# Polarisjame/DeepFake

Measured on AMD Instinct MI355X. Metric: train clips/sec (32x224x224 video + 16kHz audio) at 1/2/4/8 MI355X, higher is better.
Workload: dtype bf16; 1 GPU; C2: Swin-T video 32x224x224 (window 8x7x7) + SwinV2 mel 224 + wav2vec2-base 4s@16kHz + FusionModel, full train step; global_batch=8, per_gpu_batch=8, parallelism=dp1, hip_graph=True, captured_overlap=False, captured_bn_broadcast=False, branch_streams=3, regularisers=True

## Files before the change

### deepfake_amd/_lib.py

```python
import ctypes as C
import os

import torch

_HERE = os.path.dirname(os.path.abspath(__file__))
LIB_PATH = os.environ.get("DFK_LIB") or os.path.join(_HERE, "libdfk.so")

F32, BF16 = 0, 1


class Drop(C.Structure):
    _fields_ = [("rng", C.c_void_p), ("mode", C.c_int32), ("site", C.c_int32), ("p", C.c_float),
                ("group_rows", C.c_int32), ("shared", C.c_int32)]


class View(C.Structure):
    _fields_ = [("ptr", C.c_void_p), ("ld", C.c_int64), ("bs0", C.c_int64), ("bs1", C.c_int64),
                ("conv_cg", C.c_int32), ("conv_stride", C.c_int32), ("conv_pad", C.c_int32),
                ("conv_rows", C.c_int32)]


class GemmArgs(C.Structure):
    _fields_ = [("a", View), ("b", View), ("c", C.c_void_p), ("bias", C.c_void_p), ("residual", C.c_void_p),
                ("aux", C.c_void_p), ("ldc", C.c_int64), ("cbs0", C.c_int64), ("cbs1", C.c_int64),
# ... 42 lines not shown
class PilResize(C.Structure):
    _fields_ = [("H", C.c_int32), ("W", C.c_int32), ("cin", C.c_int32), ("out_h", C.c_int32), ("out_w", C.c_int32),
                ("xb", C.c_void_p), ("xk", C.c_void_p), ("kx", C.c_int32),
                ("yb", C.c_void_p), ("yk", C.c_void_p), ("ky", C.c_int32)]


class Conv2dGeo(C.Structure):
    _fields_ = [("N", C.c_int32), ("H", C.c_int32), ("W", C.c_int32), ("C", C.c_int32), ("kh", C.c_int32),
                ("kw", C.c_int32), ("sh", C.c_int32), ("sw", C.c_int32), ("ph", C.c_int32), ("pw", C.c_int32),
                ("Ho", C.c_int32), ("Wo", C.c_int32)]


class Im2colArgs(C.Structure):
    _fields_ = [("sb", C.c_int64), ("sc", C.c_int64), ("st", C.c_int64), ("sh", C.c_int64), ("sw", C.c_int64),
                ("B", C.c_int32), ("cin", C.c_int32), ("T", C.c_int32), ("H", C.c_int32), ("W", C.c_int32),
                ("pd", C.c_int32), ("ph", C.c_int32), ("pw", C.c_int32),
                ("Do", C.c_int32), ("Ho", C.c_int32), ("Wo", C.c_int32)]


_VP, _I64, _I32, _F = C.c_void_p, C.c_int64, C.c_int32, C.c_float
SIGNATURES = {
    "dfk_gemm": [C.POINTER(GemmArgs), _VP],
    "dfk_gemm_workspace": [C.POINTER(GemmArgs)],
    "dfk_colsum": [_VP, C.c_int, _I64, _I64, _I64, _VP, _VP],
    "dfk_gemm_mx": [C.POINTER(GemmArgs), C.POINTER(MxOperand), C.POINTER(MxOperand), _VP],
    "dfk_mx_quant": [_VP, C.c_int, _I64, _I64, _I64, C.c_int, _VP, _I64, _VP, _VP],
    "dfk_layernorm_fwd": [_VP, _VP, _VP, _VP, _VP, _VP, _I64, _I32, _F, C.c_int, _VP, C.POINTER(Drop), _VP],
    "dfk_layernorm_bwd": [_VP, _VP, _VP, _VP, _VP, _VP, _VP, _VP, _I64, _I32, C.c_int, C.c_int, _VP,
                          C.POINTER(Drop), _VP, _VP],
    "dfk_layernorm_bwd_workspace": [_I64, _I32],
    "dfk_wattn_fwd": [C.POINTER(WattnArgs), _VP],
    "dfk_wattn_bwd": [C.POINTER(WattnBwdArgs), _VP],
    "dfk_wattn_bwd_workspace": [C.POINTER(WattnArgs)],
    "dfk_wattn_fwd_policy": [C.c_int32, C.c_int64],
    "dfk_wattn_bwd_policy": [C.c_int32, C.c_int32],
    "dfk_wattn_table_workspace": [C.POINTER(WattnArgs)],
    "dfk_wattn_table": [C.POINTER(WattnArgs), _VP],
    "dfk_patch_im2col": [_VP, C.c_int, _VP, C.c_int, C.POINTER(Im2colArgs), _VP],
    "dfk_patch_merge": [_VP, _VP, C.c_int, C.c_int, C.c_int, C.c_int, C.c_int, C.c_int, C.c_int, _VP],
    "dfk_rowmean": [_VP, _VP, C.c_int, C.c_int, C.c_int, C.c_int, C.c_int, _VP],
    "dfk_cast": [_VP, C.c_int, _VP, C.c_int, _I64, _VP],
    "dfk_gelu_bwd": [_VP, _VP, _VP, _I64, C.c_int, _VP],
    "dfk_posconv_wnorm_fwd": [_VP, _VP, C.c_int32, C.c_int32, C.c_int32, _VP, _VP, _VP, _VP, C.c_int, _VP],
    "dfk_posconv_wnorm_bwd": [_VP, _VP, _VP, _VP, C.c_int32, C.c_int32, C.c_int32, _VP, _VP, _VP, _VP],
    "dfk_cosine_qk_fwd": [_VP, _VP, _VP, _F, _I64, C.c_int, C.c_int, C.c_int, _VP],
    "dfk_cosine_qk_bwd": [_VP, _VP, _VP, _VP, _F, _VP, _I64, C.c_int, C.c_int, C.c_int, _VP, _VP],
# ... 112 lines not shown
```

### deepfake_amd/csrc/gemm.hip

```cpp
#include <mutex>

#include "common.h"

namespace {

constexpr int NT = 256;

struct SplitK {
  float* slab;
  uint32_t* cnt;
};

template <typename T> struct GT;
template <> struct GT<bf16raw> { static constexpr int BK = 64, VEC = 8, PADR = 8, PADK = 16; };
template <> struct GT<float> { static constexpr int BK = 32, VEC = 4, PADR = 4, PADK = 4; };

template <typename T, bool KMAJ, int ROWS>
struct Tile {
  static constexpr int TBK = GT<T>::BK;
  static constexpr int STRIDE = KMAJ ? ROWS + GT<T>::PADK : TBK + GT<T>::PADR;
  static constexpr int ELEMS = KMAJ ? TBK * STRIDE : ROWS * STRIDE;
};

template <bool CONV>
// ... 498 lines not shown
__device__ __forceinline__ bf16x8 frag_dma(const bf16raw* img, int r0, int kb, int lane) {
  if constexpr (!KM) {
    const int r = r0 + (lane & 15), c = (kb >> 3) + (lane >> 4);
    return *reinterpret_cast<const bf16x8*>(img + r * 64 + ((c ^ ((r >> 1) & 7)) << 3));
  } else {
    const int li = lane & 15, q = li >> 2, p = li & 3;
    const int k = kb + (lane >> 4) * 8 + q, c = (r0 >> 3) + (p >> 1);
    const bf16raw* lo = img + k * ROWS + ((c ^ kmaj_swz<ROWS>(k)) << 3) + (p & 1) * 4;
    const bf16raw* hi = img + (k + 4) * ROWS + ((c ^ kmaj_swz<ROWS>(k + 4)) << 3) + (p & 1) * 4;
    const short4v a = __builtin_amdgcn_ds_read_tr16_b64_v4i16((lds_short4*)(lo));
    const short4v b = __builtin_amdgcn_ds_read_tr16_b64_v4i16((lds_short4*)(hi));
    short8 u = {a[0], a[1], a[2], a[3], b[0], b[1], b[2], b[3]};
    return __builtin_bit_cast(bf16x8, u);
  }
}

__host__ __device__ __forceinline__ long view_extent(const dfk_view& v, long rows, long cols) {
  if (v.conv_cg > 0) return ((long)(v.conv_rows - 1) * v.ld + v.conv_cg) * 2;
  return ((rows - 1) * v.ld + cols) * 2;
}

constexpr int kRsPartialMin = 32;

template <int WT, int NWM, int NWN, bool AK, bool BKM, int S, bool RS, bool CONV = false>
__global__ __launch_bounds__(NWM * NWN * 64) void gemm_dma_kernel(const dfk_gemm_args g, int kchunk, int evec,
                                                                  SplitK sk) {
  constexpr int NWV = NWM * NWN, BM = NWM * WT, BN = NWN * WT, MI = WT / 16, BK = 64;
  constexpr int STAGE = (BM + BN) * BK;
  constexpr int ES = WT + 4;
  constexpr int SMEM = S * STAGE * 2 > NWV * WT * ES * 4 ? S * STAGE * 2 : NWV * WT * ES * 4;
  constexpr int LPT = Dma<AK, BM, NWV, CONV>::NI + Dma<BKM, BN, NWV, CONV>::NI;
  __shared__ __attribute__((aligned(16))) float smem_f[SMEM / 4];
  bf16raw* smem = reinterpret_cast<bf16raw*>(smem_f);
  const int tid = threadIdx.x, lane = tid & 63;
  const int wave = __builtin_amdgcn_readfirstlane(tid >> 6);
  const int wm = wave / NWN, wn = wave % NWN;
  int tn, tmi, z;
  const int nwg = gridDim.x * gridDim.y;
  if (g.atomic && g.splitk % 8 == 0 && (int)gridDim.z == g.splitk && nwg > 1) {
    const int lin = blockIdx.z * nwg + blockIdx.y * gridDim.x + blockIdx.x;
    const int j = lin >> 3, i = j % nwg;
    z = (j / nwg) * 8 + (lin & 7);
    tn = i % gridDim.x;
    tmi = i / gridDim.x;
  } else {
    const int bid = blockIdx.y * gridDim.x + blockIdx.x;
    const int xcd = bid & 7, q = nwg >> 3, rr = nwg & 7;
    const int nid = (xcd < rr ? xcd * (q + 1) : rr * (q + 1) + (xcd - rr) * q) + (bid >> 3);
    tn = nid % gridDim.x;
    tmi = nid / gridDim.x;
    z = blockIdx.z;
  }
  const int bn = tn * BN, bm = tmi * BM;
  const int split = z % g.splitk;
  z /= g.splitk;
  const int z0 = z / g.nz1, z1 = z % g.nz1;
  const bf16raw* A = reinterpret_cast<const bf16raw*>(g.a.ptr) + z0 * g.a.bs0 + z1 * g.a.bs1;
  const bf16raw* B = reinterpret_cast<const bf16raw*>(g.b.ptr) + z0 * g.b.bs0 + z1 * g.b.bs1;
  const __amdgpu_buffer_rsrc_t ra = __builtin_amdgcn_make_buffer_rsrc(
      const_cast<bf16raw*>(A), (short)0, (int)(AK ? view_extent(g.a, g.K, g.M) : view_extent(g.a, g.M, g.K)), 0x00020000);
  const __amdgpu_buffer_rsrc_t rb = __builtin_amdgcn_make_buffer_rsrc(
      const_cast<bf16raw*>(B), (short)0, (int)(BKM ? view_extent(g.b, g.K, g.N) : view_extent(g.b, g.N, g.K)), 0x00020000);
  const int kbeg = split * kchunk;
  const int kend = min(g.K, kbeg + kchunk);
  const int ntile = kend > kbeg ? (kend - kbeg + BK - 1) / BK : 0;

  auto issue = [&](int kt, bf16raw* st) {
    Dma<AK, BM, NWV, CONV>::issue(ra, g.a, bm, g.M, kt, kend, st, wave, lane);
    Dma<BKM, BN, NWV, CONV>::issue(rb, g.b, bn, g.N, kt, kend, st + BM * BK, wave, lane);
  };

  f32x4 acc[MI][MI];
#pragma unroll
  for (int i = 0; i < MI; ++i)
// ... 54 lines not shown
    }
  }
  if (RS && do_rs && (lane & 15) == 0) {
    float* rsp = g.splitk >= kRsPartialMin && g.ws
                     ? reinterpret_cast<float*>(g.ws) + (g.atomic ? 0L : (long)g.splitk * g.M * g.N) + (long)split * g.M
                     : nullptr;
#pragma unroll
    for (int h = 0; h < MH; ++h) {
      const int mi = h * NWN + wn;
      if (mi < MI)
#pragma unroll
        for (int r = 0; r < 4; ++r) {
          const int row = bm + wm * WT + mi * 16 + (lane >> 4) * 4 + r;
          if (row < g.M) {
            if (rsp) rsp[row] = accr[h][r];
            else atomicAdd(g.rowsum + row, accr[h][r]);
          }
        }
    }
  }
  asm volatile("s_waitcnt vmcnt(0) lgkmcnt(0)" ::: "memory");
  __syncthreads();
  tile_epilogue<bf16raw, WT>(g, smem_f, acc, lane, wave, wm, wn, bm, bn, z, split,
                             (z * (int)gridDim.y + tmi) * (int)gridDim.x + tn, evec, sk);
}

__global__ __launch_bounds__(1024) void rowsum_reduce_kernel(const float* __restrict__ part, int splitk, int M,
                                                             float* __restrict__ rowsum) {
  __shared__ float red[16][64];
  const int c = threadIdx.x & 63, ph = threadIdx.x >> 6;
  const int row = blockIdx.x * 64 + c;
  float a[4] = {0.f, 0.f, 0.f, 0.f};
  if (row < M) {
    int sp = ph;
    for (; sp + 48 < splitk; sp += 64)
#pragma unroll
      for (int u = 0; u < 4; ++u) a[u] += part[(long)(sp + 16 * u) * M + row];
    for (; sp < splitk; sp += 16) a[0] += part[(long)sp * M + row];
  }
  red[ph][c] = (a[0] + a[1]) + (a[2] + a[3]);
  __syncthreads();
  if (ph == 0 && row < M) {
    float t = 0.f;
#pragma unroll
    for (int i = 0; i < 16; ++i) t += red[i][c];
    rowsum[row] += t;
  }
// ... 103 lines not shown
template <int WT, int NWM, int NWN, int S>
void dispatch_dma_s(const dfk_gemm_args& g, dim3 grid, int kchunk, int evec, SplitK sk, hipStream_t s) {
  const dim3 blk(NWM * NWN * 64);
  if (g.a_kmajor) {
    if (g.b_kmajor) {
      if (g.rowsum) hipLaunchKernelGGL((gemm_dma_kernel<WT, NWM, NWN, true, true, S, true>), grid, blk, 0, s, g, kchunk, evec, sk);
      else hipLaunchKernelGGL((gemm_dma_kernel<WT, NWM, NWN, true, true, S, false>), grid, blk, 0, s, g, kchunk, evec, sk);
    }
    else hipLaunchKernelGGL((gemm_dma_kernel<WT, NWM, NWN, true, false, S, false>), grid, blk, 0, s, g, kchunk, evec, sk);
  } else {
    if (g.b_kmajor) hipLaunchKernelGGL((gemm_dma_kernel<WT, NWM, NWN, false, true, S, false>), grid, blk, 0, s, g, kchunk, evec, sk);
    else hipLaunchKernelGGL((gemm_dma_kernel<WT, NWM, NWN, false, false, S, false>), grid, blk, 0, s, g, kchunk, evec, sk);
  }
}

int dma_stages(int wt) {
  static const int s128 = getenv("DFK_DMA_S128") ? atoi(getenv("DFK_DMA_S128")) : 2;
  if (wt == 128) return s128;
  static const int s64 = getenv("DFK_DMA_S64") ? atoi(getenv("DFK_DMA_S64")) : 2;
  static const int s32 = getenv("DFK_DMA_S32") ? atoi(getenv("DFK_DMA_S32")) : 2;
  return wt == 64 ? s64 : s32;
}

void dispatch_dma(const dfk_gemm_args& g, int wt, dim3 grid, int kchunk, int evec, SplitK sk, hipStream_t s) {
  if (g.a.conv_cg > 0 || g.b.conv_cg > 0) {
    if (wt == 32) dispatch_dma_conv<32>(g, grid, kchunk, evec, sk, s);
    else dispatch_dma_conv<64>(g, grid, kchunk, evec, sk, s);
    return;
  }
  static const int sdw = getenv("DFK_DMA_SDW") ? atoi(getenv("DFK_DMA_SDW")) : 2;
  static const int sdw32 = getenv("DFK_DMA_SDW32") ? atoi(getenv("DFK_DMA_SDW32")) : 2;
  const int st = g.a_kmajor && wt == 64 ? sdw : (g.a_kmajor && wt == 32 ? sdw32 : dma_stages(wt));
  static const int s8w = getenv("DFK_DMA_S8W") ? atoi(getenv("DFK_DMA_S8W")) : 2;
  if (wt == 33) {
    if (s8w == 3) dispatch_dma_s<32, 4, 2, 3>(g, grid, kchunk, evec, sk, s);
    else dispatch_dma_s<32, 4, 2, 2>(g, grid, kchunk, evec, sk, s);
    return;
  }
  if (wt == 34) {
    if (s8w == 3) dispatch_dma_s<32, 2, 4, 3>(g, grid, kchunk, evec, sk, s);
    else dispatch_dma_s<32, 2, 4, 2>(g, grid, kchunk, evec, sk, s);
    return;
  }
  if (wt == 128) {
    if (st == 3) dispatch_dma_s<64, 4, 2, 3>(g, grid, kchunk, evec, sk, s);
    else dispatch_dma_s<64, 4, 2, 2>(g, grid, kchunk, evec, sk, s);
  } else if (wt == 64) {
    if (st == 2) dispatch_dma_s<64, 2, 2, 2>(g, grid, kchunk, evec, sk, s);
    else if (st == 4) dispatch_dma_s<64, 2, 2, 4>(g, grid, kchunk, evec, sk, s);
    else dispatch_dma_s<64, 2, 2, 3>(g, grid, kchunk, evec, sk, s);
  } else {
    if (st == 2) dispatch_dma_s<32, 2, 2, 2>(g, grid, kchunk, evec, sk, s);
    else if (st == 4) dispatch_dma_s<32, 2, 2, 4>(g, grid, kchunk, evec, sk, s);
    else dispatch_dma_s<32, 2, 2, 3>(g, grid, kchunk, evec, sk, s);
  }
// ... 351 lines not shown
  static uint32_t* arena[64] = {};
  static long cursor[64] = {};
  std::lock_guard<std::mutex> lock(mu);
  int dev = 0;
  if (hipGetDevice(&dev) != hipSuccess || dev < 0 || dev >= 64) return nullptr;
  if (!arena[dev]) {
    void* p = nullptr;
    if (hipMalloc(&p, kTickets * 4) != hipSuccess) return nullptr;
    if (hipMemsetAsync(p, 0, kTickets * 4, s) != hipSuccess || hipStreamSynchronize(s) != hipSuccess) {
      (void)hipFree(p);
      return nullptr;
    }
    arena[dev] = static_cast<uint32_t*>(p);
  }
  if (cursor[dev] + n > kTickets) cursor[dev] = 0;
  uint32_t* t = arena[dev] + cursor[dev];
  cursor[dev] += (n + 63) & ~63L;
  return t;
}

extern "C" int dfk_gemm(const dfk_gemm_args* g, hipStream_t s) {
  if (!g || g->mx_q) return DFK_EINVAL;
  return g->dtype == DFK_BF16 ? launch<bf16raw>(*g, s) : launch<float>(*g, s);
}

extern "C" int64_t dfk_gemm_workspace(const dfk_gemm_args* g) {
  if (!g) return -1;
  const int autos = g->splitk > 1 && !g->atomic ? g->splitk
                    : (g->dtype == DFK_BF16 ? auto_splitk<bf16raw>(*g) : auto_splitk<float>(*g));
  const bool dmav = g->dtype == DFK_BF16 && dma_ok(*g) && view_vec(g->a, 8) && view_vec(g->b, 8) &&
                    (g->a_kmajor ? g->M : g->K) % 8 == 0 && (g->b_kmajor ? g->N : g->K) % 8 == 0;
  const int64_t rs = !dmav || !g->rowsum ? 0
                     : (g->atomic && g->splitk >= kRsPartialMin ? (int64_t)g->splitk * g->M * 4
                                                                : (autos >= kRsPartialMin ? (int64_t)autos * g->M * 4 : 0));
  if (autos <= 1) return rs;
  return (int64_t)autos * g->nz0 * g->nz1 * g->M * g->N * 4 + rs;
}

extern "C" int dfk_colsum(const void* x, int dtype, int64_t rows, int64_t cols, int64_t ld, float* out,
                          hipStream_t s) {
  if (!x || !out || cols <= 0) return DFK_EINVAL;
  if (rows <= 0) return 0;
  long chunks = rows < 64 ? 1 : std::min<long>(1024, (rows + 63) / 64);
  long rows_per = (rows + chunks - 1) / chunks;
  chunks = (rows + rows_per - 1) / rows_per;
  dim3 grid(dfk_cdiv(cols, 256), (unsigned)chunks);
// ... 74 lines not shown
```

### deepfake_amd/functional.py

```python
import os

import torch

from . import kernels as K


def _orig(p):
    if p is None or hasattr(p, "_dfk_store") or not isinstance(p, torch.Tensor):
        return p
    from .params import PARAM_BY_PTR
    q = PARAM_BY_PTR.get(p.data_ptr())
    return q if q is not None and q.shape == p.shape else p


def compute_weight(p, dtype):
    if p is None:
        return None
    p = _orig(p)
    if p.dtype == dtype:
        return p
    sh = getattr(p, "_dfk_shadow", None)
    if sh is not None and sh.dtype == dtype:
        return sh
    return p.detach().to(dtype)
# ... 14 lines not shown
    p = _orig(p)
    st = _store(p)
    if st is not None and ctx.needs_input_grad[idx] and not _RECOMPUTING[0]:
        st.uses[id(p)] = st.uses.get(id(p), 0) + 1


def grad_sink(p):
    p = _orig(p)
    st = _store(p)
    if st is not None:
        if p.grad is None:
            st.rebind_grads()
        return p.grad
    return _f32_zeros(p)


def grad_done(p, g):
    p = _orig(p)
    st = _store(p)
    if st is None:
        return g
    st.grad_ready(p)
    return None


def checkpoint(fn, *args):
    import contextlib
    import torch.utils.checkpoint as cp

    @contextlib.contextmanager
    def recompute():
        _RECOMPUTING[0] += 1
        try:
            yield
        finally:
            _RECOMPUTING[0] -= 1
    return cp.checkpoint(fn, *args, use_reentrant=False,
                         context_fn=lambda: (contextlib.nullcontext(), recompute()))


def rows2d(x):
    return x.reshape(-1, x.shape[-1])


def mx_weight(p, transpose=False):
    return K.mx_quant(_orig(p).detach(), transpose=transpose)
# ... 15 lines not shown
        else:
            y = K.linear(x, compute_weight(weight, dt), b, act=act, aux=aux, residual=residual, drop=drop)
        grad_use(ctx, 1, weight)
        grad_use(ctx, 2, bias)
        ctx.save_for_backward(x, weight, bias, aux)
        ctx.act, ctx.has_bias, ctx.has_res, ctx.drop, ctx.mx = act, bias is not None, residual is not None, drop, mx
        return y

    @staticmethod
    def backward(ctx, dy):
        x, weight, bias, aux = ctx.saved_tensors
        dy = dy.contiguous()
        dz = K.dropout(dy, ctx.drop) if ctx.drop is not None else dy
        dz = K.gelu_bwd(dz, aux) if ctx.act == 1 else dz
        dx = None
        if ctx.needs_input_grad[0]:
            if ctx.mx:
                dx = K.gemm_mx(K.mx_quant(dz), mx_weight(weight, transpose=True))
            else:
                dx = K.linear_dx(dz, compute_weight(weight, x.dtype))
        dw = db = None
        want_b = ctx.has_bias and ctx.needs_input_grad[2]
        if ctx.needs_input_grad[1]:
            db = grad_sink(bias) if want_b else None
            dw = grad_done(weight, K.linear_dw(dz, x, grad_sink(weight), db=db))
        elif want_b:
            db = K.colsum(dz, grad_sink(bias))
        if want_b:
            db = grad_done(bias, db)
        return dx, dw, db, None, (dy if ctx.has_res else None), None, None


def linear(x, weight, bias=None, act=0, residual=None, drop=None, mx=False):
    shp = x.shape
    x2 = rows2d(x).contiguous()
    y = LinearFn.apply(x2, weight, bias, act, rows2d(residual).contiguous() if residual is not None else None, drop,
                       mx_ok(x2, weight, mx))
    return y.view(*shp[:-1], weight.shape[0])


class GroupLinearFn(torch.autograd.Function):

    @staticmethod
    def forward(ctx, x, st, wspan, wshape, bspan, skip, *params):
        dt = x.dtype
        src = st.shadow if (dt == torch.bfloat16 and st.shadow is not None) else st.flat
        if src.dtype != dt:
            raise RuntimeError("GroupLinearFn: compute dtype has no flat view")
        W = src[wspan[0]:wspan[0] + wspan[1]].view(wshape)
        B = src[bspan[0]:bspan[0] + bspan[1]] if bspan is not None else None
        y = K.linear(x, W, B)
        for i, p in enumerate(params):
            grad_use(ctx, 6 + i, p)
        ctx.save_for_backward(x, *params)
        ctx.st, ctx.wspan, ctx.wshape, ctx.bspan, ctx.skip = st, wspan, wshape, bspan, skip
        if skip:
            return y, x.view_as(x)
        return y

    @staticmethod
    def backward(ctx, dy, dskip=None):
        x, *params = ctx.saved_tensors
        st, (wo, wn), wshape, bspan = ctx.st, ctx.wspan, ctx.wshape, ctx.bspan
        dy = dy.contiguous()
        src = st.shadow if (x.dtype == torch.bfloat16 and st.shadow is not None) else st.flat
        dx = K.linear_dx(dy, src[wo:wo + wn].view(wshape), residual=dskip if ctx.skip else None) \
            if ctx.needs_input_grad[0] else None
        if any(p.grad is None for p in params):
            st.rebind_grads()
        db = st.grad[bspan[0]:bspan[0] + bspan[1]] if bspan is not None else None
        K.linear_dw(dy, x, st.grad[wo:wo + wn].view(wshape), db=db)
        for p in params:
            grad_done(p, None)
        return (dx, None, None, None, None, None) + (None,) * len(params)


def linear_group(x, weights, biases=None, skip=False):
    shp = x.shape
    x2 = rows2d(x).contiguous()
    st = _store(weights[0])
    if st is not None:
        ws = st.group_span(list(weights))
        bs = st.group_span(list(biases)) if biases is not None else None
        if ws is not None and (biases is None or bs is not None):
            wshape = (sum(w.shape[0] for w in weights), weights[0].shape[1])
            ps = list(weights) + [b for b in (biases or []) if not isinstance(b, int)]
            out = GroupLinearFn.apply(x2, st, ws, wshape, bs, skip, *ps)
            if skip:
                return out[0].view(*shp[:-1], wshape[0]), out[1].view(shp)
            return out.view(*shp[:-1], wshape[0])
    W = torch.cat(list(weights)) if len(weights) > 1 else weights[0]
    b = None
    if biases is not None:
        b = torch.cat([torch.zeros(e, device=x.device, dtype=weights[0].dtype) if isinstance(e, int) else e
                       for e in biases])
    y = linear(x, W, b)
# ... 27 lines not shown
        ctx.res_is_input, ctx.skip, ctx.mx = res_is_input, skip, mx
        if skip:
            return y, x.view_as(x)
        return y

    @staticmethod
    def backward(ctx, dy, dskip=None):
        x, w1, b1, w2, b2, pre, h = ctx.saved_tensors
        dy = dy.contiguous()
        dyr = dy
        if ctx.drop_out is not None:
            dy = K.dropout(dy, ctx.drop_out)
        dt = x.dtype
        extra = dyr if ctx.res_is_input else (dskip if ctx.skip else None)
        if ctx.mx:
            dpre, dpreq = K.gemm_mx(K.mx_quant(dy), mx_weight(w2, transpose=True), act=2, aux=pre, drop=ctx.drop_act,
                                    mx_out=True)
            dx = K.gemm_mx(dpreq, mx_weight(w1, transpose=True),
                           residual=extra.contiguous() if extra is not None else None) \
                if ctx.needs_input_grad[0] else None
        else:
            dpre = K.linear_dx(dy, compute_weight(w2, dt), act=2, aux=pre, drop=ctx.drop_act)
            dx = K.linear_dx(dpre, compute_weight(w1, dt), residual=extra) if ctx.needs_input_grad[0] else None
        db2 = grad_sink(b2)
        dw2 = grad_done(w2, K.linear_dw(dy, h, grad_sink(w2), db=db2))
        db2 = grad_done(b2, db2)
        db1 = grad_sink(b1)
        dw1 = grad_done(w1, K.linear_dw(dpre, x, grad_sink(w1), db=db1))
        db1 = grad_done(b1, db1)
        dres = dyr if (ctx.has_res and not ctx.res_is_input) else None
        return dx, dw1, db1, dw2, db2, dres, None, None, None, None, None


def mlp(x, fc1, fc2, residual=None, drop_act=None, drop_out=None, skip=False, mx=False):
    shp = x.shape
    x2 = rows2d(x).contiguous()
    res_is_input = residual is not None and residual is x
    r2 = x2 if res_is_input else (rows2d(residual).contiguous() if residual is not None else None)
    mx = mx_ok(x2, fc1.weight, mx) and fc2.weight.shape[0] % 128 == 0
    out = MlpFn.apply(x2, fc1.weight, fc1.bias, fc2.weight, fc2.bias, r2, drop_act, drop_out, res_is_input, skip, mx)
    if skip:
        y, xs = out
        return y.view(*shp[:-1], fc2.weight.shape[0]), xs.view(shp)
    return out.view(*shp[:-1], fc2.weight.shape[0])


class LayerNormFn(torch.autograd.Function):

    @staticmethod
    def forward(ctx, x, weight, bias, eps, residual=None, drop=None, skip=False):
        dt = x.dtype
        y, mean, rstd = K.layernorm_fwd(x, compute_weight(weight, dt), compute_weight(bias, dt), eps,
# ... 606 lines not shown
```

### deepfake_amd/kernels.py

```python
import ctypes
import math
import os

import torch

from . import _lib as L

_CU_TARGET_BLOCKS = int(os.environ.get("DFK_DW_TARGET", "256"))


def _view(t, ld, bs0=0, bs1=0, conv=None):
    v = L.View()
    v.ptr = t.data_ptr()
    v.ld, v.bs0, v.bs1 = int(ld), int(bs0), int(bs1)
    if conv:
        v.conv_cg, v.conv_stride, v.conv_pad, v.conv_rows = (int(c) for c in conv)
    return v


def gemm(a, a_ld, a_kmajor, b, b_ld, b_kmajor, M, N, K, c, ldc, *, dtype, c_f32=False, bias=None,
         residual=None, ldr=0, aux=None, ldaux=0, act=0, beta=0.0, atomic=False, splitk=1,
         nz=(1, 1), a_bs=(0, 0), b_bs=(0, 0), c_bs=(0, 0), r_bs=(0, 0), a_conv=None, b_conv=None, bias_bs1=0,
         rowsum=None, drop=None, alpha=0.0):
    g = L.GemmArgs()
    if drop is not None:
        g.drop = L.drop(drop, c.device)
    g.bias_bs1 = int(bias_bs1)
    g.a = _view(a, a_ld, *a_bs, conv=a_conv)
    g.b = _view(b, b_ld, *b_bs, conv=b_conv)
    g.c = c.data_ptr()
    g.bias = bias.data_ptr() if bias is not None else None
    g.residual = residual.data_ptr() if residual is not None else None
    g.aux = aux.data_ptr() if aux is not None else None
    g.ldc, g.cbs0, g.cbs1 = int(ldc), int(c_bs[0]), int(c_bs[1])
    g.ldr, g.rbs0, g.rbs1 = int(ldr), int(r_bs[0]), int(r_bs[1])
    g.ldaux = int(ldaux)
    g.M, g.N, g.K = int(M), int(N), int(K)
    g.dtype = dtype
    g.a_kmajor, g.b_kmajor = int(a_kmajor), int(b_kmajor)
    g.c_f32 = int(c_f32)
    g.nz0, g.nz1 = int(nz[0]), int(nz[1])
    g.splitk = int(splitk)
    g.act = int(act)
    g.atomic = int(atomic)
    g.beta = float(beta)
    g.rowsum = rowsum.data_ptr() if rowsum is not None else None
    g.alpha = float(alpha)
    for t in (a, b, c):
        if not t.is_cuda:
            raise RuntimeError("deepfake_amd: tensors must be on the HIP device (no CPU fallback)")
    ws = None
    nbytes = L.lib().dfk_gemm_workspace(g)
    if nbytes > 0:
        ws = torch.empty(nbytes // 4, device=c.device, dtype=torch.float32)
        g.ws = ws.data_ptr()
    L.check(L.lib().dfk_gemm(g, L.stream()), f"gemm M={M} N={N} K={K}")


def linear(x, w, b=None, act=0, aux=None, residual=None, out=None, beta=0.0, drop=None):
    M, K = x.shape
    N = w.shape[0]
    if out is None:
        out = torch.empty(M, N, device=x.device, dtype=x.dtype)
    gemm(x, x.stride(0), False, w, w.stride(0), False, M, N, K, out, out.stride(0), dtype=L.dt(x), bias=b,
         residual=residual, ldr=residual.stride(0) if residual is not None else 0, aux=aux,
         ldaux=aux.stride(0) if aux is not None else 0, act=act, beta=beta, drop=drop)
    return out


class MxTensor:

    def __init__(self, q, s):
        self.q, self.s = q, s

    @property
    def shape(self):
        return tuple(self.q.shape)

    def operand(self):
# ... 68 lines not shown
        residual = residual.contiguous()
    if (_DX_BLAS and act == 0 and beta == 0.0 and drop is None and residual is None and M <= _DX_BLAS_MAX_M
            and dy.dtype == torch.bfloat16 and w.dtype == torch.bfloat16 and dy.is_contiguous() and out.is_contiguous()):
        return torch.matmul(dy, w, out=out)
    gemm(dy, dy.stride(0), False, w, w.stride(0), True, M, K, N, out, out.stride(0), dtype=L.dt(dy), act=act,
         aux=aux, ldaux=aux.stride(0) if aux is not None else 0, beta=beta, drop=drop, residual=residual,
         ldr=residual.stride(0) if residual is not None else 0)
    return out


_DX_BLAS = os.environ.get("DFK_DX_BLAS", "1") == "1"
_DX_BLAS_MAX_M = int(os.environ.get("DFK_DX_BLAS_MAX_M", "131072"))
_DW_MIN_K = int(os.environ.get("DFK_DW_MINK", "512"))
_DW_UNSPLIT64 = int(os.environ.get("DFK_DW_UNSPLIT64", "384"))
_DW_XCD = int(os.environ.get("DFK_DW_XCD", "1"))
_DW_SLAB = os.environ.get("DFK_DW_SLAB", "0") == "1"


def splitk_for(tiles, K, min_k=None):
    min_k = _DW_MIN_K if min_k is None else min_k
    return max(1, min(_CU_TARGET_BLOCKS // max(tiles, 1), max(K // min_k, 1)))


def linear_dw(dy, x, dw, db=None):
    M, N = dy.shape
    K = x.shape[1]
    if math.ceil(N / 64) * math.ceil(K / 64) >= _DW_UNSPLIT64:
        gemm(dy, dy.stride(0), True, x, x.stride(0), True, N, K, M, dw, dw.stride(0), dtype=L.dt(dy), c_f32=True,
             beta=1.0, rowsum=db)
        return dw
    tiles = math.ceil(N / 128) * math.ceil(K / 128)
    s = splitk_for(tiles, M)
    s = max(1, min(s, max(8, M * (N + K) // (8 * N * K))))
    if _DW_XCD and tiles > 1 and s >= 16:
        s -= s % 8
    slab = s > 1 and _DW_SLAB
    gemm(dy, dy.stride(0), True, x, x.stride(0), True, N, K, M, dw, dw.stride(0), dtype=L.dt(dy), c_f32=True,
         atomic=s > 1 and not slab, beta=1.0, splitk=s, rowsum=db)
    return dw


def colsum(x, out):
    rows, cols = x.shape
    L.check(L.lib().dfk_colsum(L.ptr(x), L.dt(x), rows, cols, x.stride(0), L.ptr(out), L.stream()), "colsum")
    return out


def layernorm_fwd(x, w, b, eps=1e-5, out=None, residual=None, drop=None):
    rows, C = x.shape
    if out is None:
        out = torch.empty_like(x)
    mean = torch.empty(rows, device=x.device, dtype=torch.float32)
    rstd = torch.empty(rows, device=x.device, dtype=torch.float32)
    d = L.drop(drop, x.device)
    L.check(L.lib().dfk_layernorm_fwd(L.ptr(x), L.ptr(w), L.ptr(b), L.ptr(out), L.ptr(mean), L.ptr(rstd), rows, C,
                                      float(eps), L.dt(x), L.ptr(residual), d, L.stream()), "layernorm_fwd")
    return out, mean, rstd


_LN_SMALL = int(os.environ.get("DFK_LN_SMALL", "128"))
_LN_SMALL_ROWS = 4096

# ... 515 lines not shown
```

### deepfake_amd/trainer.py

```python
import contextlib
import math
import os
import time

import torch
import torch.distributed as dist

from . import rng
from .ddp import GradBucketer, fr_last_id, recorder_on
from .optim import CosineAnnealingLR, FusedAdamW, FusedSGD, ParamEMA
from .params import ParamStore
from .utils import AverageMeter, Logger


def pad_longest(waves, return_lengths=False):
    if torch.is_tensor(waves):
        out = waves.float()
        return (out, torch.full((out.shape[0],), out.shape[-1], dtype=torch.int64)) if return_lengths else out
    arrs = [torch.as_tensor(w, dtype=torch.float32).reshape(-1) for w in waves]
    S = max(a.numel() for a in arrs)
    out = torch.zeros(len(arrs), S, dtype=torch.float32)
    for i, a in enumerate(arrs):
        out[i, :a.numel()] = a
    if return_lengths:
        return out, torch.tensor([a.numel() for a in arrs], dtype=torch.int64)
    return out


def normalize_wave(w):
    from . import kernels as K
# ... 79 lines not shown
        self.ema = ema
        if parallel_branches and hasattr(model, "parallel_branches") and torch.cuda.is_available() \
                and store.flat.is_cuda:
            model.parallel_branches = True
            bucketer.streams = model.branch_streams()
        self.lossF = torch.nn.BCELoss()
        self.graph_mode = graph
        self.graph = None
        self.static = None
        self.captured_overlap = None
        self.captured_bn = False
        self.agraphs = None
        self.first_micro = True
        if not bucketer.bn_buffers:
            bucketer.track_batchnorm(model)

    def _fwd_bwd(self, feature, label, scale=1.0, before_backward=None):
        rng.advance(self.store.flat.device)
        prob = self.model(feature)
        loss = self.lossF(prob.float().reshape(-1), label.float().reshape(-1))
        if before_backward is not None:
            before_backward()
        (loss * scale if scale != 1.0 else loss).backward()
        if getattr(self.model, "parallel_branches", False):
            self.model.join_branches()
        return loss, prob

    def micro(self, feature, label, last, accum=1):
        if self.graph_mode and accum > 1:
            return self._micro_graphed(feature, label, last, accum)
        return self._micro_eager(feature, label, last, accum)

    def _micro_eager(self, feature, label, last, accum):
        if self.first_micro:
            self.bucketer.broadcast_bn()
            self.first_micro = False
        if not last:
            with self.bucketer.no_sync():
                loss, prob = self._fwd_bwd(feature, label, 1.0 / accum)
            return loss.detach(), prob.detach()
        loss, prob = self._fwd_bwd(feature, label, 1.0 / accum)
        fold = self._fold()
        fa = self.bucketer.finish(fold=fold)
        self.opt.step(**fa)
        if self.ema is not None:
            self.ema.update()
# ... 359 lines not shown
```

### include/dfk.h

```cpp
#ifndef DFK_H
#define DFK_H
#include <stdint.h>
#include <hip/hip_runtime.h>

#ifdef __cplusplus
extern "C" {
#endif

#define DFK_F32 0
#define DFK_BF16 1
#define DFK_EINVAL (-1)
#define DFK_ENOTSUP (-2)

typedef struct {
  const int64_t* rng;
  int32_t mode;
  int32_t site;
  float p;
  int32_t group_rows;
  int32_t shared;
} dfk_drop;

typedef struct {
  const void* ptr;
// ... 16 lines not shown
  int64_t ldc, cbs0, cbs1;
  int64_t ldr, rbs0, rbs1;
  int64_t ldaux;
  int64_t bias_bs1;
  int32_t M, N, K;
  int32_t dtype;
  int32_t a_kmajor, b_kmajor;
  int32_t c_f32;
  int32_t nz0, nz1;
  int32_t splitk;
  int32_t act;
  int32_t atomic;
  float beta;
  void* ws;
  float* rowsum;
  dfk_drop drop;
  float alpha;
  uint8_t* mx_q;
  uint32_t* mx_s;
  int64_t mx_ldq, mx_lds;
} dfk_gemm_args;
int dfk_gemm(const dfk_gemm_args* g, hipStream_t stream);
int64_t dfk_gemm_workspace(const dfk_gemm_args* g);

typedef struct {
  const uint8_t* q;
  const uint32_t* s;
  int64_t ld;
  int64_t lds;
} dfk_mx_operand;
int dfk_mx_quant(const void* x, int dtype, int64_t rows, int64_t cols, int64_t ldx, int transpose, uint8_t* q,
                 int64_t ldq, uint32_t* s, hipStream_t stream);
int dfk_gemm_mx(const dfk_gemm_args* g, const dfk_mx_operand* a, const dfk_mx_operand* b, hipStream_t stream);

int dfk_colsum(const void* x, int dtype, int64_t rows, int64_t cols, int64_t ld, float* out, hipStream_t stream);

int dfk_layernorm_fwd(const void* x, const void* w, const void* b, void* y, float* mean, float* rstd,
                      int64_t rows, int32_t C, float eps, int dtype, const void* residual, const dfk_drop* drop,
                      hipStream_t stream);
int dfk_layernorm_bwd(const void* dy, const void* x, const void* w, const float* mean, const float* rstd,
                      void* dx, float* dw, float* db, int64_t rows, int32_t C, int accumulate, int dtype,
                      float* ws, const dfk_drop* drop, const void* addend, hipStream_t stream);
int64_t dfk_layernorm_bwd_workspace(int64_t rows, int32_t C);

typedef struct {
  const void* q; const void* k; const void* v;
// ... 216 lines not shown
```

Before: 286.7 clips/s.

## Batch small weight-gradient GEMMs into grouped persistent launches

Weight-gradient GEMMs for small linear layers are now deferred into a per-stream queue and flushed as one grouped kernel. Each block looks up its problem from a table passed as kernel arguments, so up to eight dW GEMMs share a single launch. The GEMM kernel body is factored into a device function taking explicit block and grid indices. The aim is to cut per-launch overhead and fill the GPU better when individual dW GEMMs are too small to occupy it. The cost is delayed gradient-ready callbacks, which may reduce overlap with gradient communication, plus extra Python bookkeeping and a flush at the end of backward.

```diff
diff --git a/deepfake_amd/_lib.py b/deepfake_amd/_lib.py
--- a/deepfake_amd/_lib.py
+++ b/deepfake_amd/_lib.py
@@ -88,6 +88,7 @@
 SIGNATURES = {
     "dfk_gemm": [C.POINTER(GemmArgs), _VP],
     "dfk_gemm_workspace": [C.POINTER(GemmArgs)],
+    "dfk_gemm_dw_group": [C.POINTER(GemmArgs), _I32, _VP],
     "dfk_colsum": [_VP, C.c_int, _I64, _I64, _I64, _VP, _VP],
     "dfk_gemm_mx": [C.POINTER(GemmArgs), C.POINTER(MxOperand), C.POINTER(MxOperand), _VP],
     "dfk_mx_quant": [_VP, C.c_int, _I64, _I64, _I64, C.c_int, _VP, _I64, _VP, _VP],
diff --git a/deepfake_amd/csrc/gemm.hip b/deepfake_amd/csrc/gemm.hip
--- a/deepfake_amd/csrc/gemm.hip
+++ b/deepfake_amd/csrc/gemm.hip
@@ -544,9 +544,9 @@
 
 constexpr int kRsPartialMin = 32;
 
-template <int WT, int NWM, int NWN, bool AK, bool BKM, int S, bool RS, bool CONV = false>
-__global__ __launch_bounds__(NWM * NWN * 64) void gemm_dma_kernel(const dfk_gemm_args g, int kchunk, int evec,
-                                                                  SplitK sk) {
+template <int WT, int NWM, int NWN, bool AK, bool BKM, int S, bool RS, bool CONV>
+__device__ __forceinline__ void gemm_dma_body(const dfk_gemm_args& g, int kchunk, int evec, SplitK sk, const dim3 bid,
+                                              const dim3 grid) {
   constexpr int NWV = NWM * NWN, BM = NWM * WT, BN = NWN * WT, MI = WT / 16, BK = 64;
   constexpr int STAGE = (BM + BN) * BK;
   constexpr int ES = WT + 4;
@@ -558,20 +558,20 @@
   const int wave = __builtin_amdgcn_readfirstlane(tid >> 6);
   const int wm = wave / NWN, wn = wave % NWN;
   int tn, tmi, z;
-  const int nwg = gridDim.x * gridDim.y;
-  if (g.atomic && g.splitk % 8 == 0 && (int)gridDim.z == g.splitk && nwg > 1) {
-    const int lin = blockIdx.z * nwg + blockIdx.y * gridDim.x + blockIdx.x;
+  const int nwg = grid.x * grid.y;
+  if (g.atomic && g.splitk % 8 == 0 && (int)grid.z == g.splitk && nwg > 1) {
+    const int lin = bid.z * nwg + bid.y * grid.x + bid.x;
     const int j = lin >> 3, i = j % nwg;
     z = (j / nwg) * 8 + (lin & 7);
-    tn = i % gridDim.x;
-    tmi = i / gridDim.x;
+    tn = i % grid.x;
+    tmi = i / grid.x;
   } else {
-    const int bid = blockIdx.y * gridDim.x + blockIdx.x;
-    const int xcd = bid & 7, q = nwg >> 3, rr = nwg & 7;
-    const int nid = (xcd < rr ? xcd * (q + 1) : rr * (q + 1) + (xcd - rr) * q) + (bid >> 3);
-    tn = nid % gridDim.x;
-    tmi = nid / gridDim.x;
-    z = blockIdx.z;
+    const int b2 = bid.y * grid.x + bid.x;
+    const int xcd = b2 & 7, q = nwg >> 3, rr = nwg & 7;
+    const int nid = (xcd < rr ? xcd * (q + 1) : rr * (q + 1) + (xcd - rr) * q) + (b2 >> 3);
+    tn = nid % grid.x;
+    tmi = nid / grid.x;
+    z = bid.z;
   }
   const int bn = tn * BN, bm = tmi * BM;
   const int split = z % g.splitk;
@@ -672,7 +672,62 @@
   asm volatile("s_waitcnt vmcnt(0) lgkmcnt(0)" ::: "memory");
   __syncthreads();
   tile_epilogue<bf16raw, WT>(g, smem_f, acc, lane, wave, wm, wn, bm, bn, z, split,
-                             (z * (int)gridDim.y + tmi) * (int)gridDim.x + tn, evec, sk);
+                             (z * (int)grid.y + tmi) * (int)grid.x + tn, evec, sk);
+}
+
+template <int WT, int NWM, int NWN, bool AK, bool BKM, int S, bool RS, bool CONV = false>
+__global__ __launch_bounds__(NWM * NWN * 64) void gemm_dma_kernel(const dfk_gemm_args g, int kchunk, int evec,
+                                                                  SplitK sk) {
+  gemm_dma_body<WT, NWM, NWN, AK, BKM, S, RS, CONV>(g, kchunk, evec, sk, blockIdx, gridDim);
+}
+
+constexpr int kDwGroupMax = 8;
+struct DwProblem {
+  const void *a, *b;
+  float *c, *rowsum;
+  int32_t M, N, K;
+  int32_t lda, ldb, ldc;
+  int32_t splitk, kchunk;
+  int32_t gx, gy;
+};
+struct DwGroup {
+  DwProblem p[kDwGroupMax];
+  int32_t prefix[kDwGroupMax + 1];
+  int32_t n;
+};
+static_assert(sizeof(DwGroup) + 64 <= 4096, "the problem table must fit the kernel-argument block");
+
+template <int WT, bool RS>
+__global__ __launch_bounds__(256) void gemm_dw_group_kernel(const DwGroup T) {
+  const int b = blockIdx.x;
+  int pi = 0;
+#pragma unroll
+  for (int i = 1; i < kDwGroupMax; ++i) pi += (i < T.n && b >= T.prefix[i]) ? 1 : 0;
+  pi = __builtin_amdgcn_readfirstlane(pi);
+  const DwProblem& P = T.p[pi];
+  const int local = __builtin_amdgcn_readfirstlane(b - T.prefix[pi]);
+  const int gx = P.gx, gy = P.gy, gz = P.splitk;
+  if (local >= gx * gy * gz) return;
+  dfk_gemm_args g{};
+  g.a.ptr = P.a;
+  g.a.ld = P.lda;
+  g.b.ptr = P.b;
+  g.b.ld = P.ldb;
+  g.c = P.c;
+  g.ldc = P.ldc;
+  g.M = P.M;
+  g.N = P.N;
+  g.K = P.K;
+  g.dtype = DFK_BF16;
+  g.a_kmajor = g.b_kmajor = g.c_f32 = 1;
+  g.nz0 = g.nz1 = 1;
+  g.splitk = P.splitk;
+  g.atomic = P.splitk > 1;
+  g.beta = 1.f;
+  g.rowsum = P.rowsum;
+  const int xy = gx * gy;
+  const dim3 bid(local % gx, (local % xy) / gx, local / xy), grid(gx, gy, gz);
+  gemm_dma_body<WT, 2, 2, true, true, 2, RS, false>(g, P.kchunk, 0, SplitK{nullptr, nullptr}, bid, grid);
 }
 
 __global__ __launch_bounds__(1024) void rowsum_reduce_kernel(const float* __restrict__ part, int splitk, int M,
@@ -822,15 +877,19 @@
   return wt == 64 ? s64 : s32;
 }
 
+int dw_stages(int wt) {
+  static const int sdw = getenv("DFK_DMA_SDW") ? atoi(getenv("DFK_DMA_SDW")) : 2;
+  static const int sdw32 = getenv("DFK_DMA_SDW32") ? atoi(getenv("DFK_DMA_SDW32")) : 2;
+  return wt == 64 ? sdw : sdw32;
+}
+
 void dispatch_dma(const dfk_gemm_args& g, int wt, dim3 grid, int kchunk, int evec, SplitK sk, hipStream_t s) {
   if (g.a.conv_cg > 0 || g.b.conv_cg > 0) {
     if (wt == 32) dispatch_dma_conv<32>(g, grid, kchunk, evec, sk, s);
     else dispatch_dma_conv<64>(g, grid, kchunk, evec, sk, s);
     return;
   }
-  static const int sdw = getenv("DFK_DMA_SDW") ? atoi(getenv("DFK_DMA_SDW")) : 2;
-  static const int sdw32 = getenv("DFK_DMA_SDW32") ? atoi(getenv("DFK_DMA_SDW32")) : 2;
-  const int st = g.a_kmajor && wt == 64 ? sdw : (g.a_kmajor && wt == 32 ? sdw32 : dma_stages(wt));
+  const int st = g.a_kmajor && (wt == 64 || wt == 32) ? dw_stages(wt) : dma_stages(wt);
   static const int s8w = getenv("DFK_DMA_S8W") ? atoi(getenv("DFK_DMA_S8W")) : 2;
   if (wt == 33) {
     if (s8w == 3) dispatch_dma_s<32, 4, 2, 3>(g, grid, kchunk, evec, sk, s);
@@ -1228,6 +1287,90 @@
 extern "C" int dfk_gemm(const dfk_gemm_args* g, hipStream_t s) {
   if (!g || g->mx_q) return DFK_EINVAL;
   return g->dtype == DFK_BF16 ? launch<bf16raw>(*g, s) : launch<float>(*g, s);
+}
+
+bool dw_group_plan(const dfk_gemm_args& g, DwProblem& r, int& wt) {
+  if (g.dtype != DFK_BF16 || !g.a_kmajor || !g.b_kmajor || !g.c_f32 || g.mx_q) return false;
+  if (!g.a.ptr || !g.b.ptr || !g.c || g.M <= 0 || g.N <= 0 || g.K <= 0) return false;
+  if (g.nz0 != 1 || g.nz1 != 1 || g.a.conv_cg > 0 || g.b.conv_cg > 0) return false;
+  if (g.bias || g.residual || g.aux || g.act || g.drop.mode || (g.alpha != 0.f && g.alpha != 1.f)) return false;
+  if (g.splitk < 1 || (g.atomic != 0) != (g.splitk > 1) || (!g.atomic && g.beta != 1.f)) return false;
+  if (g.rowsum && g.splitk >= kRsPartialMin) return false;
+  if (g.K >= 16384) return false;
+  if (!dma_ok(g) || !view_vec(g.a, 8) || !view_vec(g.b, 8) || g.M % 8 || g.N % 8) return false;
+  if (g.a.ld > 0x7fffffffL || g.b.ld > 0x7fffffffL || g.ldc > 0x7fffffffL) return false;
+  if (auto_splitk<bf16raw>(g) != 1 || getenv("DFK_GEMM_T256") || getenv("DFK_GEMM_T32X")) return false;
+  wt = pick_wt(g);
+  if ((wt != 32 && wt != 64) || dw_stages(wt) != 2) return false;
+  const long gx = dfk_cdiv(g.N, 2 * wt), gy = dfk_cdiv(g.M, 2 * wt);
+  if (gy > 65535 || g.splitk > 65535 || gx * gy * g.splitk > (1L << 24)) return false;
+  r.a = g.a.ptr;
+  r.b = g.b.ptr;
+  r.c = reinterpret_cast<float*>(g.c);
+  r.rowsum = g.rowsum;
+  r.M = g.M, r.N = g.N, r.K = g.K;
+  r.lda = (int32_t)g.a.ld, r.ldb = (int32_t)g.b.ld, r.ldc = (int32_t)g.ldc;
+  r.splitk = g.splitk;
+  r.kchunk = dfk_cdiv(dfk_cdiv(g.K, g.splitk), 64) * 64;
+  r.gx = (int32_t)gx, r.gy = (int32_t)gy;
+  return true;
+}
+
+static bool ranges_meet(const void* p, long n, const void* q, long m) {
+  const uintptr_t a = reinterpret_cast<uintptr_t>(p), b = reinterpret_cast<uintptr_t>(q);
+  return p && q && a < b + (uintptr_t)m && b < a + (uintptr_t)n;
+}
+
+extern "C" int dfk_gemm_dw_group(const dfk_gemm_args* problems, int32_t n, hipStream_t s) {
+  if (n < 0 || (n > 0 && !problems)) return DFK_EINVAL;
+  DwGroup T[4] = {};
+  int32_t first[4] = {0, 0, 0, 0};
+  auto flush = [&](int k) -> int {
+    DwGroup& G = T[k];
+    const int m = G.n;
+    if (m == 0) return 0;
+    if (m == 1) {
+      G.n = 0;
+      return dfk_gemm(&problems[first[k]], s);
+    }
+    const dim3 grid((unsigned)G.prefix[m]), blk(256);
+    if (k == 0) hipLaunchKernelGGL((gemm_dw_group_kernel<32, false>), grid, blk, 0, s, G);
+    else if (k == 1) hipLaunchKernelGGL((gemm_dw_group_kernel<32, true>), grid, blk, 0, s, G);
+    else if (k == 2) hipLaunchKernelGGL((gemm_dw_group_kernel<64, false>), grid, blk, 0, s, G);
+    else hipLaunchKernelGGL((gemm_dw_group_kernel<64, true>), grid, blk, 0, s, G);
+    G.n = 0;
+    DFK_CHECK_LAUNCH();
+    return 0;
+  };
+  for (int i = 0; i < n; ++i) {
+    const dfk_gemm_args& g = problems[i];
+    DwProblem r;
+    int wt = 0;
+    if (n == 1 || !dw_group_plan(g, r, wt)) {
+      for (int k = 0; k < 4; ++k)
+        if (const int rc = flush(k)) return rc;
+      if (const int rc = dfk_gemm(&g, s)) return rc;
+      continue;
+    }
+    const int k = (wt == 64 ? 2 : 0) + (r.rowsum ? 1 : 0);
+    DwGroup& G = T[k];
+    const long cb = ((long)(r.M - 1) * r.ldc + r.N) * 4, rb = (long)r.M * 4;
+    bool clash = false;
+    for (int j = 0; j < G.n; ++j) {
+      const DwProblem& o = G.p[j];
+      clash = clash || ranges_meet(r.c, cb, o.c, ((long)(o.M - 1) * o.ldc + o.N) * 4) ||
+              ranges_meet(r.rowsum, rb, o.rowsum, (long)o.M * 4);
+    }
+    if (clash || G.n == kDwGroupMax)
+      if (const int rc = flush(k)) return rc;
+    if (G.n == 0) { first[k] = i; G.prefix[0] = 0; }
+    G.p[G.n] = r;
+    G.prefix[G.n + 1] = G.prefix[G.n] + (r.gx * r.gy * r.splitk + 7) / 8 * 8;
+    ++G.n;
+  }
+  for (int k = 0; k < 4; ++k)
+    if (const int rc = flush(k)) return rc;
+  return 0;
 }
 
 extern "C" int64_t dfk_gemm_workspace(const dfk_gemm_args* g) {
diff --git a/deepfake_amd/functional.py b/deepfake_amd/functional.py
--- a/deepfake_amd/functional.py
+++ b/deepfake_amd/functional.py
@@ -60,6 +60,22 @@
         return g
     st.grad_ready(p)
     return None
+
+
+def linear_dw_params(dy, x, weight, bias=None, dw=None, db=None, params=None):
+    ps = params if params is not None else [p for p in (weight, bias) if p is not None]
+    if dw is None:
+        dw = grad_sink(weight)
+        db = grad_sink(bias) if bias is not None else None
+    if all(_store(p) is not None for p in ps):
+        def done():
+            for p in ps:
+                grad_done(p, None)
+        if K.linear_dw(dy, x, dw, db=db, defer=True, done=done) is True and K.dw_pending() == 1:
+            torch.autograd.Variable._execution_engine.queue_callback(K.dw_flush_all)
+        return None, None
+    K.linear_dw(dy, x, dw, db=db)
+    return grad_done(weight, dw), (grad_done(bias, db) if bias is not None else None)
 
 
 def checkpoint(fn, *args):
@@ -121,12 +137,9 @@
         dw = db = None
         want_b = ctx.has_bias and ctx.needs_input_grad[2]
         if ctx.needs_input_grad[1]:
-            db = grad_sink(bias) if want_b else None
-            dw = grad_done(weight, K.linear_dw(dz, x, grad_sink(weight), db=db))
+            dw, db = linear_dw_params(dz, x, weight, bias if want_b else None)
         elif want_b:
-            db = K.colsum(dz, grad_sink(bias))
-        if want_b:
-            db = grad_done(bias, db)
+            db = grad_done(bias, K.colsum(dz, grad_sink(bias)))
         return dx, dw, db, None, (dy if ctx.has_res else None), None, None
 
 
@@ -168,9 +181,8 @@
         if any(p.grad is None for p in params):
             st.rebind_grads()
         db = st.grad[bspan[0]:bspan[0] + bspan[1]] if bspan is not None else None
-        K.linear_dw(dy, x, st.grad[wo:wo + wn].view(wshape), db=db)
-        for p in params:
-            grad_done(p, None)
+        linear_dw_params(dy, x, None, dw=st.grad[wo:wo + wn].view(wshape), db=db, params=[_orig(p) for p in params])
+        K.dw_flush()
         return (dx, None, None, None, None, None) + (None,) * len(params)
 
 
@@ -244,12 +256,8 @@
         else:
             dpre = K.linear_dx(dy, compute_weight(w2, dt), act=2, aux=pre, drop=ctx.drop_act)
             dx = K.linear_dx(dpre, compute_weight(w1, dt), residual=extra) if ctx.needs_input_grad[0] else None
-        db2 = grad_sink(b2)
-        dw2 = grad_done(w2, K.linear_dw(dy, h, grad_sink(w2), db=db2))
-        db2 = grad_done(b2, db2)
-        db1 = grad_sink(b1)
-        dw1 = grad_done(w1, K.linear_dw(dpre, x, grad_sink(w1), db=db1))
-        db1 = grad_done(b1, db1)
+        dw2, db2 = linear_dw_params(dy, h, w2, b2)
+        dw1, db1 = linear_dw_params(dpre, x, w1, b1)
         dres = dyr if (ctx.has_res and not ctx.res_is_input) else None
         return dx, dw1, db1, dw2, db2, dres, None, None, None, None, None
 
diff --git a/deepfake_amd/kernels.py b/deepfake_amd/kernels.py
--- a/deepfake_amd/kernels.py
+++ b/deepfake_amd/kernels.py
@@ -22,6 +22,16 @@
          residual=None, ldr=0, aux=None, ldaux=0, act=0, beta=0.0, atomic=False, splitk=1,
          nz=(1, 1), a_bs=(0, 0), b_bs=(0, 0), c_bs=(0, 0), r_bs=(0, 0), a_conv=None, b_conv=None, bias_bs1=0,
          rowsum=None, drop=None, alpha=0.0):
+    _gemm_launch(_gemm_args(a, a_ld, a_kmajor, b, b_ld, b_kmajor, M, N, K, c, ldc, dtype=dtype, c_f32=c_f32, bias=bias,
+                            residual=residual, ldr=ldr, aux=aux, ldaux=ldaux, act=act, beta=beta, atomic=atomic,
+                            splitk=splitk, nz=nz, a_bs=a_bs, b_bs=b_bs, c_bs=c_bs, r_bs=r_bs, a_conv=a_conv,
+                            b_conv=b_conv, bias_bs1=bias_bs1, rowsum=rowsum, drop=drop, alpha=alpha), c)
+
+
+def _gemm_args(a, a_ld, a_kmajor, b, b_ld, b_kmajor, M, N, K, c, ldc, *, dtype, c_f32=False, bias=None,
+               residual=None, ldr=0, aux=None, ldaux=0, act=0, beta=0.0, atomic=False, splitk=1,
+               nz=(1, 1), a_bs=(0, 0), b_bs=(0, 0), c_bs=(0, 0), r_bs=(0, 0), a_conv=None, b_conv=None, bias_bs1=0,
+               rowsum=None, drop=None, alpha=0.0):
     g = L.GemmArgs()
     if drop is not None:
         g.drop = L.drop(drop, c.device)
@@ -49,12 +59,16 @@
     for t in (a, b, c):
         if not t.is_cuda:
             raise RuntimeError("deepfake_amd: tensors must be on the HIP device (no CPU fallback)")
+    return g
+
+
+def _gemm_launch(g, c):
     ws = None
     nbytes = L.lib().dfk_gemm_workspace(g)
     if nbytes > 0:
         ws = torch.empty(nbytes // 4, device=c.device, dtype=torch.float32)
         g.ws = ws.data_ptr()
-    L.check(L.lib().dfk_gemm(g, L.stream()), f"gemm M={M} N={N} K={K}")
+    L.check(L.lib().dfk_gemm(g, L.stream()), f"gemm M={g.M} N={g.N} K={g.K}")
 
 
 def linear(x, w, b=None, act=0, aux=None, residual=None, out=None, beta=0.0, drop=None):
@@ -169,22 +183,95 @@
     return max(1, min(_CU_TARGET_BLOCKS // max(tiles, 1), max(K // min_k, 1)))
 
 
-def linear_dw(dy, x, dw, db=None):
+_DW_GROUP = [int(os.environ.get("DFK_DW_GROUP", "1"))]
+_DW_GROUP_MAX = 8
+_DW_GROUP_BLOCKS = 768
+_DW_GROUP_BYTES = 32 << 20
+_dw_queues = {}
+
+
+def dw_group_policy(n):
+    dw_flush_all()
+    old, _DW_GROUP[0] = _DW_GROUP[0], int(n)
+    return old
+
+
+def dw_pending():
+    return sum(len(q) for _, q in _dw_queues.values())
+
+
+def dw_flush():
+    ent = _dw_queues.pop(torch.cuda.current_stream().cuda_stream, None)
+    if not ent or not ent[1]:
+        return
+    q = ent[1]
+    arr = (L.GemmArgs * len(q))(*[e[0] for e in q])
+    L.check(L.lib().dfk_gemm_dw_group(arr, len(q), L.stream()), f"gemm_dw_group n={len(q)}")
+    for _, _, done in q:
+        if done is not None:
+            done()
+
+
+def dw_flush_all():
+    for key in list(_dw_queues):
+        ent = _dw_queues.get(key)
+        if ent is not None:
+            with torch.cuda.stream(ent[0]):
+                dw_flush()
+
+
+def linear_dw_group(problems):
+    gs, keep = [], []
+    for dy, x, dw, db in problems:
+        g, _ = _dw_args(dy, x, dw, db)
+        nbytes = L.lib().dfk_gemm_workspace(g)
+        if nbytes > 0:
+            keep.append(torch.empty(nbytes // 4, device=dw.device, dtype=torch.float32))
+            g.ws = keep[-1].data_ptr()
+        gs.append(g)
+    if gs:
+        arr = (L.GemmArgs * len(gs))(*gs)
+        L.check(L.lib().dfk_gemm_dw_group(arr, len(gs), L.stream()), f"gemm_dw_group n={len(gs)}")
+
+
+def linear_dw(dy, x, dw, db=None, defer=False, done=None):
+    g, blocks = _dw_args(dy, x, dw, db)
+    M, N = dy.shape
+    K = x.shape[1]
+    if (defer and _DW_GROUP[0] and blocks < _DW_GROUP_BLOCKS and M * (N + K) * 2 <= _DW_GROUP_BYTES
+            and dy.dtype == torch.bfloat16 and L.lib().dfk_gemm_workspace(g) == 0):
+        cur = torch.cuda.current_stream()
+        q = _dw_queues.setdefault(cur.cuda_stream, (cur, []))[1]
+        q.append((g, (dy, x, dw, db), done))
+        if len(q) >= _DW_GROUP_MAX:
+            dw_flush()
+        return True
+    if _dw_queues:
+        dw_flush()
+    _gemm_launch(g, dw)
+    if done is not None:
+        done()
+    return dw
+
+
+def _dw_args(dy, x, dw, db):
     M, N = dy.shape
     K = x.shape[1]
     if math.ceil(N / 64) * math.ceil(K / 64) >= _DW_UNSPLIT64:
-        gemm(dy, dy.stride(0), True, x, x.stride(0), True, N, K, M, dw, dw.stride(0), dtype=L.dt(dy), c_f32=True,
-             beta=1.0, rowsum=db)
-        return dw
-    tiles = math.ceil(N / 128) * math.ceil(K / 128)
-    s = splitk_for(tiles, M)
-    s = max(1, min(s, max(8, M * (N + K) // (8 * N * K))))
-    if _DW_XCD and tiles > 1 and s >= 16:
-        s -= s % 8
-    slab = s > 1 and _DW_SLAB
-    gemm(dy, dy.stride(0), True, x, x.stride(0), True, N, K, M, dw, dw.stride(0), dtype=L.dt(dy), c_f32=True,
-         atomic=s > 1 and not slab, beta=1.0, splitk=s, rowsum=db)
-    return dw
+        blocks = math.ceil(N / 64) * math.ceil(K / 64)
+        g = _gemm_args(dy, dy.stride(0), True, x, x.stride(0), True, N, K, M, dw, dw.stride(0), dtype=L.dt(dy),
+                       c_f32=True, beta=1.0, rowsum=db)
+    else:
+        tiles = math.ceil(N / 128) * math.ceil(K / 128)
+        s = splitk_for(tiles, M)
+        s = max(1, min(s, max(8, M * (N + K) // (8 * N * K))))
+        if _DW_XCD and tiles > 1 and s >= 16:
+            s -= s % 8
+        slab = s > 1 and _DW_SLAB
+        blocks = tiles * s
+        g = _gemm_args(dy, dy.stride(0), True, x, x.stride(0), True, N, K, M, dw, dw.stride(0), dtype=L.dt(dy),
+                       c_f32=True, atomic=s > 1 and not slab, beta=1.0, splitk=s, rowsum=db)
+    return g, blocks
 
 
 def colsum(x, out):
diff --git a/deepfake_amd/trainer.py b/deepfake_amd/trainer.py
--- a/deepfake_amd/trainer.py
+++ b/deepfake_amd/trainer.py
@@ -6,6 +6,7 @@
 import torch
 import torch.distributed as dist
 
+from . import kernels as K
 from . import rng
 from .ddp import GradBucketer, fr_last_id, recorder_on
 from .optim import CosineAnnealingLR, FusedAdamW, FusedSGD, ParamEMA
@@ -131,6 +132,7 @@
         if before_backward is not None:
             before_backward()
         (loss * scale if scale != 1.0 else loss).backward()
+        K.dw_flush_all()
         if getattr(self.model, "parallel_branches", False):
             self.model.join_branches()
         return loss, prob
diff --git a/include/dfk.h b/include/dfk.h
--- a/include/dfk.h
+++ b/include/dfk.h
@@ -62,6 +62,7 @@
 } dfk_gemm_args;
 int dfk_gemm(const dfk_gemm_args* g, hipStream_t stream);
 int64_t dfk_gemm_workspace(const dfk_gemm_args* g);
+int dfk_gemm_dw_group(const dfk_gemm_args* problems, int32_t n, hipStream_t stream);
 
 typedef struct {
   const uint8_t* q;
```

Result: faster. 297.5 clips/s, median of 6 (+3.7%).
